# p-m-mueller/saddle_point_petsc

Measured on AMD Instinct MI355X. Metric: FGMRES iterations/sec + achieved HBM GB/s on A-block SpMV, 1/2/4/8 MI355X, higher is better.
Workload: dtype f64

## Files before the change

include/spk.h:

```cpp
#ifndef SPK_H
#define SPK_H

#include <stdint.h>

#ifdef __cplusplus
extern "C" {
#endif

#define SPK_VERSION 100

typedef struct spk_ctx spk_ctx;

enum { SPK_OK = 0, SPK_ERR_ARG = -1, SPK_ERR_HIP = -2, SPK_ERR_STATE = -3,
       SPK_ERR_COMM = -4, SPK_ERR_NOMEM = -5, SPK_ERR_UNSUPPORTED = -6 };

enum { SPK_MEM_HOST = 0, SPK_MEM_DEVICE = 1 };

enum { SPK_BLOCK_A00 = 0, SPK_BLOCK_A10 = 1 };

enum { SPK_PC_NONE = 0, SPK_PC_JACOBI = 1, SPK_PC_SCHUR = 2 };
enum { SPK_SCHUR_DIAG = 0, SPK_SCHUR_LOWER = 1, SPK_SCHUR_UPPER = 2, SPK_SCHUR_FULL = 3 };
enum { SPK_ORTHOG_CGS = 0, SPK_ORTHOG_MGS = 1 };
enum { SPK_REFINE_NEVER = 0, SPK_REFINE_IFNEEDED = 1, SPK_REFINE_ALWAYS = 2 };
enum { SPK_SPMV_CSR = 0 };
// ... 7 lines not shown
    int32_t restart;
    int32_t max_it;
    double rtol;
    double abstol;
    double dtol;
    int32_t guess_nonzero;
    int32_t orthog;
    int32_t check_every;
    int32_t fused;
    int32_t cgs_refine;
    int32_t single_reduce;
    int32_t iteration_form;
    int32_t reserved;
} spk_opts;
enum { SPK_ITER_AUTO = 0, SPK_ITER_FOUR_LAUNCH = 1, SPK_ITER_TWO_LAUNCH = 2, SPK_ITER_THREE_LAUNCH = 3, SPK_ITER_BA = 4,
       SPK_ITER_UNNORM = 5, SPK_ITER_RESIDENT = 6, SPK_ITER_LAST = 6 };

typedef struct spk_result {
    int32_t its;
    int32_t reason;
    double rnorm;
    double rnorm0;
    int32_t hist_len;
    int32_t cycles;
    double solve_seconds;
} spk_result;

int spk_create(spk_ctx **ctx, int device);
int spk_destroy(spk_ctx *ctx);
const char *spk_last_error(const spk_ctx *ctx);
int spk_version(void);
// ... 96 lines not shown
```

saddle_point_petsc_amd/csrc/spk_device.hpp:

```cpp
#pragma once
#include "spk_internal.hpp"

#include <cmath>
#include <cstdlib>

namespace spk {
namespace k {

constexpr int kThreads = 256;
constexpr int kWave = 64;
constexpr int kVT = 1024;
constexpr int kVWaves = kVT / kWave;
constexpr int kVecUnroll = 4;
constexpr int kVecMaxBlocks = 256;

__device__ __forceinline__ double wave_sum(double v)
{
#pragma unroll
    for (int off = kWave / 2; off > 0; off >>= 1) v += __shfl_down(v, off, kWave);
    return v;
}

typedef double dbl2v __attribute__((ext_vector_type(2)));
typedef int int4v __attribute__((ext_vector_type(4)));
// ... 353 lines not shown
    bool on;
};
inline WsShape ws_shape(int64_t n2)
{
    WsShape v;
    static const int knob = [] { const char *e = getenv("SPK_VEC_WS"); return e ? atoi(e) : -1; }();
    v.on = n2 < (int64_t)kVecMaxBlocks * 2048 && knob != 0;
    v.U = n2 >= (int64_t)kVecMaxBlocks * 64 * 8 ? 8 : (n2 >= (int64_t)kVecMaxBlocks * 64 * 4 ? 4 : 2);
    if (knob == 2 || knob == 4 || knob == 8) v.U = knob;
    int64_t tiles = (n2 + 64 * v.U - 1) / (64 * v.U);
    if (tiles < 1) tiles = 1;
    v.grid = (int)(tiles < kVecMaxBlocks ? tiles : kVecMaxBlocks);
    return v;
}

struct VecShape {
    int T, U, grid, G;
};
inline VecShape vec_shape(int64_t n2, bool maxpy = false)
{
    VecShape v;
    v.G = 4;
    int cap = kVecMaxBlocks;
    if (n2 >= (int64_t)kVecMaxBlocks * 2048) { v.T = 512; v.U = 4; }
    else if (n2 >= (int64_t)kVecMaxBlocks * 1024) { v.T = 256; v.U = 4; }
    else if (n2 >= (int64_t)kVecMaxBlocks * 512) { v.T = 256; v.U = 2; }
    else { v.T = 256; v.U = 1; }
    if (maxpy && n2 < (int64_t)kVecMaxBlocks * 1024) { v.T = 256; v.U = 1; v.G = 8; cap = 1024; }
    else if (maxpy && n2 < (int64_t)kVecMaxBlocks * 2048) { v.T = 256; v.U = 2; v.G = 8; cap = 1024; }
    int64_t tiles = (n2 + (int64_t)v.T * v.U - 1) / ((int64_t)v.T * v.U);
// ... 15 lines not shown
```

saddle_point_petsc_amd/csrc/spk_internal.hpp:

```cpp
#pragma once
#include <hip/hip_runtime.h>

#include <cstdint>
#include <cstdio>
#include <functional>
#include <memory>
#include <string>
#include <vector>

#include <hip/hip_ext.h>

#include "../../include/spk.h"

namespace spk {

struct Error {
    int code;
    std::string msg;
};
[[noreturn]] void fail(int code, const char *fmt, ...);

#define SPK_HIP(call)                                                                  \
    do {                                                                               \
        hipError_t e_ = (call);                                                        \
// ... 448 lines not shown
    double *c;
    const double *wl_in;
    int lam_in_dot;
    double *partials, *out;
    PeerAR ar;
    int32_t *err;
    uint32_t fin_ticks;
    SendRanges sr;
    int gmain;
    const int32_t *done;
    double *sc, *hbuf, *wl_out;
    KrylovArrays ka;
    int loc;
    int defer_fin;
};
void iter_spmv_mdot(const IterA &a, hipStream_t s, bool dots = true);
struct IterBA {
    const int32_t *browptr, *bcol;
    const double *vtop, *vbot;
    const int32_t *tile_brow;
    const int32_t *tdesc;
    int ntiles, tiles_per_xcd, slots, tb;
    int chunk;
    const int32_t *nbr, *wt;
    uint32_t *flags;
    uint32_t seq;
    const double *V;
    int64_t ldv;
    int nv;
    const double *dots;
// ... 126 lines not shown
    spk::k::Finish fin(double *out) { return spk::k::Finish{partials.p, out, spk::k::PeerAR{}, errw.p, fin_ticks}; }
    spk::k::Finish fin(double *out, const spk::k::PeerAR &ar) { return spk::k::Finish{partials.p, out, ar, errw.p, fin_ticks}; }
    void check_device_error();
    spk::DevBuf<double> y1tmp, ttmp;

    int last_form = -1, last_single = 0;

    int ws_restart = -1;
    spk::DevBuf<double> V, Z, xsol, rhs, tmp;
    spk::DevBuf<double> zun;
    spk::DevBuf<uint32_t> ba_flags;
    spk::DevBuf<double> ba_sc;
    spk::DevBuf<double> res_P;
    int num_cus = 0;
    uint32_t ba_seq = 0;
    spk::DevBuf<double> kry_d;
    spk::DevBuf<spk::KrylovState> kst;
    spk::k::KrylovArrays ka{};

    spk::DevBuf<double> stage_x, stage_y;

    void ensure_scratch();
    void ensure_vectors();
    void upload_staged(void *dst, const void *src, size_t bytes);
    void *pin_state = nullptr;
    hipEvent_t state_ev = nullptr;
    void *pin[2] = {nullptr, nullptr};
    hipEvent_t pin_ev[2] = {nullptr, nullptr};
};

// ... 12 lines not shown
```

saddle_point_petsc_amd/csrc/spk_k_iter.hip:

```cpp
#include "spk_device.hpp"

namespace spk {
namespace k {

template <int VW, int MINW>
__global__ __launch_bounds__(kThreads, MINW) void iter_spmv_mdot_kernel(IterA a)
{
    const int32_t dn = __builtin_nontemporal_load(a.done);
    __shared__ double prod[kBTile * 4];
    __shared__ double wt[kThreads], vt[kThreads];
    const double scale = a.nrm2 ? inv_norm(a.nrm2[0]) : 1.0;
    const int nmain = 8 * a.slots;
    const int nv = a.nv, m = a.m;
    const int scalar_wg = VW > 0 ? nmain : 0;
    const int bid = VW > 0 ? (int)blockIdx.x : (int)blockIdx.x - 1;
    if ((int)blockIdx.x == scalar_wg) {
        if (dn) return;
        double *lamw = wt;
        if ((int)threadIdx.x < m) {
            const int r = threadIdx.x;
            double wl;
            if (a.nrm2) {
                a.vcur[a.nl + r] *= scale;
                a.zdst[a.nl + r] = a.zsrc[a.nl + r] * scale;
// ... 195 lines not shown
    const int np = a.packed ? a.m / 2 : a.m;
    const int per = (a.nv + np + 3) / 4;
    if (a.nv + a.m > kMaxNv - 1) fail(SPK_ERR_ARG, "iter_spmv_mdot: %d values exceed one reduction", a.nv + a.m);
    static const int occ8 = [] { const char *e = getenv("SPK_ITERA_OCC"); return e ? atoi(e) : 4; }();
    const int occ = !dots ? 0 : (per <= 4 ? 4 : (per <= 8 ? (occ8 == 4 ? 4 : 3) : 2));
    a.slots = !dots ? (a.tiles_per_xcd > 0 ? a.tiles_per_xcd : 1) : iter_slots(a.tiles_per_xcd, occ);
    const dim3 grid(8 * a.slots + 1), block(kThreads);
    if (!dots) hipLaunchKernelGGL((iter_spmv_mdot_kernel<0, 4>), grid, block, 0, s, a);
    else if (per <= 4) hipLaunchKernelGGL((iter_spmv_mdot_kernel<4, 4>), grid, block, 0, s, a);
    else if (per <= 8 && occ8 == 4) hipLaunchKernelGGL((iter_spmv_mdot_kernel<8, 4>), grid, block, 0, s, a);
    else if (per <= 8) hipLaunchKernelGGL((iter_spmv_mdot_kernel<8, 3>), grid, block, 0, s, a);
    else if (per <= 12) hipLaunchKernelGGL((iter_spmv_mdot_kernel<12, 2>), grid, block, 0, s, a);
    else hipLaunchKernelGGL((iter_spmv_mdot_kernel<16, 2>), grid, block, 0, s, a);
}

template <int T, int G, int U, int MP>
__global__ __launch_bounds__(T) void iter_maxpy_uhead_kernel(IterB b)
{
    const int32_t dn = __builtin_nontemporal_load(b.done);
    __shared__ double hs[kMaxNv], lam[kMaxNv * 8], ys[8], wraws[8], tus[8];
    __shared__ double red[T];
    const int nv = b.nv, m = b.m;
    constexpr int NP = MP > 0 ? MP : 1;
    const int gmain = b.gmain;
    const int nhalo = b.sr.peer ? (2 * b.sr.nrecv + T - 1) / T : 0;
    const bool is_main = (int)blockIdx.x < gmain;
    const int64_t n2 = b.nl / 2;
    const int bid = blockIdx.x;
    const int bx = b.sr.peer ? ((bid & 1) ? gmain - 1 - (bid >> 1) : (bid >> 1)) : bid;

    constexpr bool PRE = U * (MP > 0 ? MP : 1) <= 16;
    double2 wv[U], dv[U], pe[PRE ? NP : 1][U], t0[G][U];
    int64_t idx[U];
    bool ok[U];
    int64_t tile = bx;
    auto load_planes = [&]() {
#pragma unroll
        for (int q = 0; q < NP; ++q) {
            const bool live = b.packed ? 2 * q < m : q < m;
#pragma unroll
// ... 24 lines not shown
    bool have = is_main && tile * (T * U) < n2;
    if (have) load_tile(tile);

    double lamv = 0.0;
    const bool lam_mine = (int)threadIdx.x < nv * m;
    if (lam_mine) lamv = b.V[(size_t)(threadIdx.x / m) * b.ldv + b.nl + (threadIdx.x % m)];
    double wl = 0.0, sh = 1.0;
    if ((int)threadIdx.x < m) {
        wl = b.wl_in[threadIdx.x];
        sh = b.shat[threadIdx.x];
    }
    double hi_pre = 0.0, qv_pre = 0.0, tbv_pre[8], sci = 1.0;
    const double s_w = b.sc ? b.sc[nv - 1] : 1.0;
    if (threadIdx.x < kWave) {
        const int i = threadIdx.x;
        hi_pre = i < nv ? b.dots[i] : 0.0;
        if (b.sc) sci = i < nv ? b.sc[i] : 0.0;
#pragma unroll
        for (int r = 0; r < 8; ++r) tbv_pre[r] = (r < m && i < nv) ? b.tb[i * 8 + r] : 0.0;
        qv_pre = (i < m) ? b.dots[nv + i] : 0.0;
    }
    if (dn) return;
    if (threadIdx.x < kWave) {
        const int i = threadIdx.x;
        const double hi = b.sc ? sci * s_w * hi_pre : hi_pre;
        const double ci = b.sc ? hi * sci : hi;
        double tbv[8];
#pragma unroll
        for (int r = 0; r < 8; ++r) tbv[r] = tbv_pre[r] * (b.sc ? sci : 1.0);
        const double qv = qv_pre * s_w;
        if (i < nv) hs[i] = ci;
        if (b.sc && (int)blockIdx.x == gmain + nhalo && i < nv) b.hbuf[i] = hi;
#pragma unroll
        for (int r = 0; r < 8; ++r) {
            if (r < m) {
                const double tsum = wave_sum(hi * tbv[r]);
                const double qr = __shfl(qv, r, kWave);
                if (i == 0) tus[r] = qr - tsum;
            }
        }
    }
    if (lam_mine) lam[threadIdx.x] = lamv;
    for (int t = threadIdx.x + T; t < nv * m; t += T) lam[t] = b.V[(size_t)(t / m) * b.ldv + b.nl + (t % m)];
    __syncthreads();
    if ((int)threadIdx.x < NP && MP > 0) {
        const int r = threadIdx.x;
        double y = 0.0, wraw = 0.0;
// ... 5 lines not shown
        wraws[r] = wraw;
        ys[r] = y;
    }
    __syncthreads();
    double yv[NP];
#pragma unroll
    for (int r = 0; r < NP; ++r) yv[r] = MP > 0 ? ys[r] : 0.0;
    if (b.sc && have) {
#pragma unroll
        for (int u = 0; u < U; ++u) {
            wv[u].x *= s_w;
            wv[u].y *= s_w;
        }
    }

    if ((int)blockIdx.x == gmain + nhalo) {
        if ((int)threadIdx.x < m) {
            const int r = threadIdx.x;
            double w1 = tus[r];
            if (b.fact == SPK_SCHUR_FULL)
                for (int q = 0; q < m; ++q) w1 -= b.gram[r * m + q] * ys[q];
            b.w[b.nl + r] = wraws[r];
            b.zun[b.nl + r] = ys[r];
            b.c[b.nl + r] = w1;
            b.tb[(size_t)nv * 8 + r] = tus[r];
            if (b.sc) b.wl_out[r] = w1;
        }
        __syncthreads();
        double lam2 = 0.0;
        if (threadIdx.x == 0)
            for (int r = 0; r < m; ++r) lam2 += b.lam_in_dot ? wraws[r] * wraws[r] : 0.0;
        if (b.defer_fin) {
            if (threadIdx.x == 0) publish(b.partials + (size_t)gmain * kPartialLd, lam2);
            return;
        }
        final_reduce(b.partials, gmain, kPartialLd, 1, red, FinErr{b.err, b.fin_ticks});
        if (threadIdx.x == 0) red[0] = red[0] + lam2;
        __syncthreads();
        if (b.ar.P) peer_allreduce_block(b.ar, red, 1, b.out);
        else if (threadIdx.x == 0) b.out[0] = red[0];
        return;
    }
    if (!is_main) {
        const int64_t g = (int64_t)((int)blockIdx.x - gmain) * T + threadIdx.x;
        if (g < 2 * (int64_t)b.sr.nrecv) {
            uint32_t lo;
            const unsigned long long tw0 = (b.sr.stats && threadIdx.x == 0) ? wall_clock64() : 0ull;
            const bool okw = granule_wait(b.sr.mine + g, b.sr.seq, b.sr.timeout_ms, lo, b.sr.err, b.done);
            if (b.sr.stats && threadIdx.x == 0) {
                atomicAdd(b.sr.stats + 2 * kStatHalo, wall_clock64() - tw0);
                atomicAdd(b.sr.stats + 2 * kStatHalo + 1, 1ull);
            }
            const uint32_t other = __shfl_xor(lo, 1, kWave);
            if (!(g & 1)) b.sr.xghost[g >> 1] = join_halves(lo, other);
            if (!okw) raise_comm_error(b.sr.err, 18, b.sr.seq);
        }
// ... 125 lines not shown
                    wv[u].y *= s_w;
                }
            }
        }
    }
    const int lane = threadIdx.x & 63, wave = threadIdx.x >> 6;
    const double sw = wave_sum(nrm);
    if (lane == 0) red[wave] = sw;
    __syncthreads();
    if (threadIdx.x == 0) {
        double tsum = 0.0;
#pragma unroll
        for (int j = 0; j < T / kWave; ++j) tsum += red[j];
        publish(b.partials + (size_t)bx * kPartialLd, tsum);
    }
}

int iter_maxpy_uhead(IterB b, hipStream_t s)
{
    const int64_t n2 = b.nl / 2;
    const bool thin = n2 < (int64_t)kVecMaxBlocks * 2048;
    static const int t128 = [] { const char *e = getenv("SPK_B_T128"); return e ? atoi(e) : 0; }();
    const int U = thin ? (n2 < (int64_t)kVecMaxBlocks * 1024 ? 1 : 2) : 4;
    const bool tiny = thin && U == 1 && t128 && n2 <= (int64_t)1024 * 128;
    const int T = tiny ? 128 : (thin ? 256 : 512);
    int64_t tiles = (n2 + (int64_t)T * U - 1) / ((int64_t)T * U);
    if (tiles < 1) tiles = 1;
    b.gmain = (int)std::min<int64_t>(tiles, thin ? 1024 : kVecMaxBlocks);
    int grid = b.gmain + 1;
    if (b.sr.peer) grid += (2 * b.sr.nrecv + T - 1) / T;
// ... 7 lines not shown
        if (!thin) SPK_IB(512, 4, 4, MPP);                                       \
        else if (tiny) SPK_IB(128, 8, 1, MPP);                                   \
        else if (U == 2) { if (g2 == 16) SPK_IB(256, 16, 2, MPP); else SPK_IB(256, 8, 2, MPP); } \
        else if (g1 == 32) SPK_IB(256, 32, 1, MPP);                              \
        else if (g1 == 16) SPK_IB(256, 16, 1, MPP);                              \
        else SPK_IB(256, 8, 1, MPP);                                             \
    } while (0)
    if (mp == 0) SPK_IB_MP(0);
    else if (mp == 4) SPK_IB_MP(4);
    else SPK_IB_MP(8);
#undef SPK_IB_MP
#undef SPK_IB
    return b.gmain;
}

__global__ __launch_bounds__(kWave) void tile_col_range_kernel(const int32_t *__restrict__ browptr, const int32_t *__restrict__ bcol,
                                                               const int32_t *__restrict__ tile_brow, int ntiles, int32_t *__restrict__ out)
{
    const int t = blockIdx.x;
    if (t >= ntiles) return;
    int lo = INT32_MAX, hi = -1;
    for (int q = browptr[tile_brow[t]] + (int)threadIdx.x; q < browptr[tile_brow[t + 1]]; q += kWave) {
        const int c = bcol[q];
        lo = c < lo ? c : lo;
        hi = c > hi ? c : hi;
    }
#pragma unroll
    for (int off = kWave / 2; off > 0; off >>= 1) {
        const int l2 = __shfl_down(lo, off, kWave), h2 = __shfl_down(hi, off, kWave);
        lo = l2 < lo ? l2 : lo;
// ... 339 lines not shown
```

saddle_point_petsc_amd/csrc/spk_k_vec.hip:

```cpp
#include "spk_device.hpp"

namespace spk {
namespace k {

__global__ void arm_partials_kernel(double *p, size_t n)
{
    const size_t i = (size_t)blockIdx.x * blockDim.x + threadIdx.x;
    if (i < n) p[i] = __longlong_as_double((long long)kSentinelBits);
}
void arm_partials(double *p, size_t n, hipStream_t s)
{
    hipLaunchKernelGGL(arm_partials_kernel, dim3((unsigned)((n + 255) / 256)), dim3(256), 0, s, p, n);
}

__global__ __launch_bounds__(256) void finish_probe_kernel(double *partials, double *out, FinErr fe)
{
    __shared__ double scratch[256];
    if (blockIdx.x + 1 < gridDim.x) {
        if (threadIdx.x == 0) publish(partials + (size_t)blockIdx.x * kPartialLd, 1.0);
        return;
    }
    __syncthreads();
    final_reduce(partials, gridDim.x, kPartialLd, 1, scratch, fe);
    if (threadIdx.x == 0) out[0] = scratch[0];
// ... 84 lines not shown
                       B.colidx.p, B.val.p, B.nrows, dinv, shat);
}



template <int NG, int T, int G, bool NT, int U>
__global__ __launch_bounds__(T) void mdot_kernel(const double *__restrict__ V, int64_t ldv, int nv,
                                                 const double *__restrict__ V2, int nv1,
                                                 const double *__restrict__ w, int64_t n2,
                                                 int64_t n_dot, double *__restrict__ partials,
                                                 int with_ww,
                                                 double *__restrict__ out, PeerAR ar, int split, FinErr fe,
                                                 const int32_t *__restrict__ done)
{
    if (done && *done) return;
    constexpr int NA = NG * 8 + 1, W = T / kWave, TILE2 = T * U;
    __shared__ double lds[(W * NA > T) ? W * NA : T];
    double acc[NA];
#pragma unroll
    for (int i = 0; i < NA; ++i) acc[i] = 0.0;

    for (int64_t tile = blockIdx.x; tile * TILE2 < n2; tile += gridDim.x) {
        double2 wv[U];
        int64_t idx[U];
#pragma unroll
        for (int u = 0; u < U; ++u) {
            idx[u] = tile * TILE2 + u * T + threadIdx.x;
            if (idx[u] < n2) {
                wv[u] = ld2(w, idx[u]);
                if (2 * idx[u] >= n_dot) wv[u].x = 0.0;
                if (2 * idx[u] + 1 >= n_dot) wv[u].y = 0.0;
            } else {
                wv[u].x = wv[u].y = 0.0;
                idx[u] = 0;
            }
        }
#pragma unroll
        for (int u = 0; u < U; ++u) acc[NA - 1] += wv[u].x * wv[u].x + wv[u].y * wv[u].y;
#pragma unroll
        for (int g0 = 0; g0 < NG * 8; g0 += G) {
            if (g0 < nv) {
                double2 a[G][U];
#pragma unroll
                for (int v = 0; v < G; ++v) {
                    const bool live = g0 + v < nv;
                    const int ic = live ? g0 + v : 0;
                    const int j2 = ic - nv1;
                    const double *Vi = !live ? w : (ic < nv1 ? V + (size_t)ic * ldv : V2 + (size_t)(split ? j2 >> 1 : j2) * ldv);
#pragma unroll
                    for (int u = 0; u < U; ++u) a[v][u] = ld2s<NT>(Vi, live ? idx[u] : 0);
                }
#pragma unroll
                for (int v = 0; v < G; ++v) {
                    const double mk = (g0 + v < nv) ? 1.0 : 0.0;
                    double d = 0.0;
                    if (split && g0 + v >= nv1 && g0 + v < nv) {
                        if ((g0 + v - nv1) & 1) {
#pragma unroll
                            for (int u = 0; u < U; ++u) d += a[v][u].y * wv[u].y;
                        } else {
#pragma unroll
                            for (int u = 0; u < U; ++u) d += a[v][u].x * wv[u].x;
                        }
                    } else {
#pragma unroll
                        for (int u = 0; u < U; ++u) d += a[v][u].x * wv[u].x + a[v][u].y * wv[u].y;
                    }
                    acc[g0 + v] += mk * d;
                }
            }
        }
    }
    const int lane = threadIdx.x & 63, wave = threadIdx.x >> 6;
#pragma unroll
    for (int i = 0; i < NA; ++i) {
        const double s = wave_sum(acc[i]);
        if (lane == 0) lds[wave * NA + i] = s;
    }
    __syncthreads();
    if (threadIdx.x < NA) {
        const int i = threadIdx.x;
        double s = 0.0;
#pragma unroll
        for (int j = 0; j < W; ++j) s += lds[j * NA + i];
        double *row = partials + (size_t)blockIdx.x * kPartialLd;
        if (i < nv) publish(row + i, s);
        else if (i == NA - 1 && with_ww) publish(row + nv, s);
    }
    if (!arrive_last(gridDim.x)) return;
    const int k = nv + (with_ww ? 1 : 0);
    final_reduce(partials, gridDim.x, kPartialLd, k, lds, fe);
    if (ar.P) peer_allreduce_block(ar, lds, k, out);
    else if ((int)threadIdx.x < k) out[threadIdx.x] = lds[threadIdx.x];
}

template <int VW, int U, int G, bool NT>
__global__ __launch_bounds__(256) void mdot_ws_kernel(const double *__restrict__ V, int64_t ldv, int nv,
                                                      const double *__restrict__ V2, int nv1,
                                                      const double *__restrict__ w, int64_t n2, int64_t n_dot,
                                                      double *__restrict__ partials, int with_ww, double *__restrict__ out,
                                                      PeerAR ar, int split, FinErr fe, const int32_t *__restrict__ done)
{
    if (done && *done) return;
// ... 800 lines not shown
```

saddle_point_petsc_amd/csrc/spk_ksp.cpp:

```cpp
#include <cstdio>
#include <cstdlib>
#include <cstring>
#include <string>
#include <vector>

#include "../../include/spk_ksp.h"

struct SpkKSP_s {
    spk_ctx *ctx = nullptr;
    int device = 0;
    spk_opts opts;
    int32_t pc_type = SPK_PC_NONE, schur_fact = SPK_SCHUR_FULL;
    int32_t inner_sweeps = 0;
    double inner_omega = 1.0;
    bool inner_richardson = false;
    bool have_ops = false, is_setup = false, has_B = false;
    bool ksp_type_given = false, pc_type_given = false;
    bool monitor = false, print_reason = false, view = false;
    spk_result result;
    std::vector<double> history;
    std::string err;
};

namespace {
// ... 192 lines not shown
        } else if (key == "-fieldsplit_0_ksp_max_it" || key == "-spk_inner_sweeps") {
            if (!val || !parse_int(val, &k->inner_sweeps)) return need("an integer");
            if (key == "-spk_inner_sweeps") k->inner_richardson = k->inner_sweeps > 0;
        } else if (key == "-fieldsplit_0_ksp_richardson_scale" || key == "-spk_inner_omega") {
            if (!val || !parse_double(val, &k->inner_omega)) return need("a real");
        } else if (key == "-fieldsplit_1_ksp_type") {
            if (!val) return need("a type");
            if (std::string(val) != "preonly") return bad();
        } else if (key == "-fieldsplit_0_pc_type" || key == "-fieldsplit_1_pc_type") {
            if (!val) return need("a type");
            if (std::string(val) != "jacobi") return bad();
        } else if (key == "-spk_single_reduce") {
            if (!val || !parse_int(val, &k->opts.single_reduce)) return need("an integer (0 off, 1 on)");
        } else if (key == "-spk_iteration_form") {
            if (!val || !parse_int(val, &k->opts.iteration_form) || k->opts.iteration_form < 0 || k->opts.iteration_form > SPK_ITER_LAST)
                return need("an integer 0..5 (0 automatic, 1 four / 2 two / 3 three launches per iteration, 4 BA, 5 three launches on an un-normalised basis)");
        } else if (key == "-spk_check_every") {
            if (!val || !parse_int(val, &k->opts.check_every)) return need("an integer");
        } else if (key.rfind("-ksp_", 0) == 0 || key.rfind("-pc_", 0) == 0 || key.rfind("-fieldsplit_", 0) == 0) {
            return set_err(k, SPK_ERR_UNSUPPORTED, "unknown solver option " + key);
        }
    }
    k->is_setup = false;
    return SPK_OK;
}

int SpkKSPSetUp(SpkKSP k)
{
    if (!k) return SPK_ERR_ARG;
    if (!k->ksp_type_given)
        return set_err(k, SPK_ERR_UNSUPPORTED, "KSPSetUp: no -ksp_type given; PETSc's default (gmres, left preconditioning) is "
// ... 63 lines not shown
```

saddle_point_petsc_amd/csrc/spk_solver.cpp:

```cpp
#include <algorithm>
#include <chrono>
#include <cstddef>
#include <cstdlib>
#include <cstring>
#include <numeric>

#include "spk_internal.hpp"

using namespace spk;

void spk_ctx::ensure_scratch()
{
    if (!partials.p) {
        partials.alloc((size_t)k::kMaxBlocks * k::kPartialLd);
        k::arm_partials(partials.p, partials.n, stream);
        SPK_HIP(hipStreamSynchronize(stream));
    }
    if (!errw.p) errw.alloc(4);
    if (!small.p) small.alloc(512);
    if (!y1tmp.p) y1tmp.alloc(64);
    if (!ttmp.p) ttmp.alloc(64);
}

void spk_ctx::check_device_error()
{
    if (!errw.p) return;
    int32_t e = 0;
    SPK_HIP(hipMemcpy(&e, errw.p, sizeof e, hipMemcpyDeviceToHost));
    if (!e) return;
    SPK_HIP(hipStreamSynchronize(stream));
    SPK_HIP(hipMemset(errw.p, 0, sizeof(int32_t)));
    k::arm_partials(partials.p, partials.n, stream);
    SPK_HIP(hipStreamSynchronize(stream));
    fail(SPK_ERR_HIP, "a cross-workgroup reduction timed out on the device (a workgroup never published its partial "
                      "sums within %.1f s): execution failure, the result of this call is not valid", fin_ticks / 1e8);
}

void spk_ctx::ensure_vectors()
{
    const int64_t want = ((int64_t)n_local + m + 255) / 256 * 256;
    if (want != ld) {
        ld = want;
        ws_restart = -1;
        tmp.release();
        zun.release();
        tmpb.release();
        bt_cached = nullptr;
        stage_x.release();
        stage_y.release();
        xsol.release();
// ... 1184 lines not shown
    const int bpk = fused && c->bd_packed ? 1 : 0;
    const double *bdp = fused ? (bpk ? c->bdpk.p : c->bd.p) : nullptr;
    const bool single = head && o.orthog == SPK_ORTHOG_CGS && o.cgs_refine == SPK_REFINE_NEVER &&
                        o.single_reduce == 1 && mk + c->m <= k::kMaxNv - 1;

    int form = o.iteration_form;
    if (const char *e = getenv("SPK_ITER_FORM")) {
        char *end = nullptr;
        const long f = strtol(e, &end, 10);
        if (end == e || *end || f < SPK_ITER_AUTO || f > SPK_ITER_LAST)
            fail(SPK_ERR_ARG, "SPK_ITER_FORM=%s: not an iteration form (%d..%d)", e, (int)SPK_ITER_AUTO, (int)SPK_ITER_LAST);
        form = (int)f;
    }
    if (form < SPK_ITER_AUTO || form > SPK_ITER_LAST) fail(SPK_ERR_ARG, "fgmres: unknown iteration_form %d", form);
    const bool un3 = head && !single && o.orthog == SPK_ORTHOG_CGS && o.cgs_refine == SPK_REFINE_NEVER &&
                     mk + c->m <= k::kMaxNv - 2 && (form == SPK_ITER_UNNORM || form == SPK_ITER_AUTO || form == SPK_ITER_RESIDENT);
    static const bool res_env_off = [] { const char *e = getenv("SPK_RESIDENT"); return e && !strcmp(e, "0"); }();
    const int res_planes = !fused ? 0 : (bpk ? m / 2 : m);
    const bool res_multi = c->comm->size() > 1;
    const bool res_rank_ok = !res_multi ? (c->peers.empty() && c->n_ghost == 0)
                                        : (c->res_fit_all && c->comm->fuses() && (c->peers.empty() || c->send_ranges.n > 0));
    const bool resident = un3 && (form == SPK_ITER_RESIDENT || (form == SPK_ITER_AUTO && !res_env_off)) && res_rank_ok &&
                          c->spmv_format == 1 && c->Adict.ok && c->Adict.bs == 2 && nl % 2 == 0 && mk >= (res_multi ? 3 : 2) &&
                          k::resident_fits(c->Adict, c->num_cus, mk, res_planes);
    if (resident) {
        const size_t need = (size_t)k::resident_scratch_doubles(c->num_cus, mk);
        if (c->res_P.n < need) c->res_P.alloc(need);
    }
    const bool two_ok = head && !single && o.orthog == SPK_ORTHOG_CGS && o.cgs_refine == SPK_REFINE_NEVER &&
                        c->spmv_format == 1 && c->Ab.ok && !c->Ab.long_rows && mk + c->m <= k::kMaxNv - 2;
    const bool two = two_ok && !un3 && (form == SPK_ITER_TWO_LAUNCH || form == SPK_ITER_THREE_LAUNCH);
    const bool three = two && form != SPK_ITER_TWO_LAUNCH;
    const bool ba = two_ok && form == SPK_ITER_BA && c->Ab.ba_ok && c->peers.empty() && c->comm->size() == 1 &&
                    (c->m <= 4 || 8 * c->Ab.ba_slots + 1 <= 512);
    if (ba) {
        const size_t nfl = (size_t)(8 * c->Ab.ba_slots + 1) * 32;
        if (c->ba_flags.n < nfl) {
            c->ba_flags.alloc(nfl);
            c->ba_seq = 0;
        }
    }
    if (ba || un3) {
        if (c->ba_sc.n < (size_t)mk + 2) c->ba_sc.alloc((size_t)mk + 2);
    }
    if (two && c->zun.n < (size_t)ld) c->zun.alloc((size_t)ld);
    const int lam_in_dot = c->comm->rank() == 0 ? 1 : 0;
    c->last_form = resident ? SPK_ITER_RESIDENT : ba ? SPK_ITER_BA : un3 ? SPK_ITER_UNNORM : two ? (three ? SPK_ITER_THREE_LAUNCH : SPK_ITER_TWO_LAUNCH)
                   : head ? SPK_ITER_FOUR_LAUNCH : -1;
    c->last_single = single ? 1 : 0;

    c->ka.tentative = single ? 1 : 0;
    KrylovState st{};
    int32_t errword = 0;
    int cycles = 0;
    if (!c->pin_state) SPK_HIP(hipHostMalloc(&c->pin_state, 512, hipHostMallocDefault));
    if (!c->state_ev) SPK_HIP(hipEventCreateWithFlags(&c->state_ev, hipEventDisableTiming));
    KrylovState *ps = (KrylovState *)c->pin_state;
    int32_t *pe = (int32_t *)((char *)c->pin_state + 384);
    pe[0] = pe[1] = 0;
    bool pend_check = false;
    bool finished = false;
    const int kAhead = 2;
// ... 70 lines not shown
                    r.shat = c->shat.p; r.gram = c->gram.p; r.P = c->res_P.p; r.ka = c->ka; r.sc_out = c->ba_sc.p;
                    r.err = c->errw.p; r.ticks = c->fin_ticks;
                    r.sr0 = k::SendRanges{};
                    r.sr1 = k::SendRanges{};
                    if (res_multi) {
                        r.sr0 = c->send_ranges;
                        r.sr1 = c->send_ranges;
                        if (!c->comm->resident_plan(mk + 1, c->peers.empty() ? 0 : mk - 1, r.ar, r.sr0, r.sr1, c->xghost.p))
                            fail(SPK_ERR_COMM, "fgmres: the communicator cannot carry a resident cycle (agreed at set-up, refused now)");
                        if (c->peers.empty()) r.sr0.n = r.sr1.n = 0;
                        if (c->n_ghost > 0) r.od = c->offdiag();
                    }
                    if (!k::cycle_resident(c->Adict, c->num_cus, r, done, s)) fail(SPK_ERR_STATE, "fgmres: resident cycle kernel refused its shape");
                    break;
                }
                {
                    const bool one = loc + 1 + m <= 40;
                    const bool spl = bpk && one;
                    const k::PeerAR ar = one ? c->comm->fused_allreduce(loc + 2 + (fused ? m : 0), k::kStatArDots) : k::PeerAR{};
                    k::mdot(V, ld, loc + 1, w, N, n_dot, c->fin(db, ar), done, s, fused ? (spl ? c->bdpk.p : c->bd.p) : nullptr,
                            fused ? m : 0, spl ? 1 : 0);
                    if (!ar.P) c->comm->allreduce_sum(db, loc + 2 + (fused ? m : 0), s);
                }
                if (un3) {
                    const k::PeerAR ar2 = c->comm->fused_allreduce(1, k::kStatArNorm);
                    k::IterB b{};
                    b.V = V; b.ldv = ld; b.nv = loc + 1; b.dots = db; b.tb = c->ka.tb;
                    b.w = w; b.dinv = c->dinv.p; b.bd = bdp; b.ldb = ld; b.shat = c->shat.p; b.gram = c->gram.p;
                    b.fact = fused ? c->schur_fact : SPK_SCHUR_LOWER;
                    b.nl = nl; b.m = m; b.packed = bpk;
                    b.zun = Zj(loc + 1); b.c = fused ? Vj(loc + 2) : nullptr; b.wl_in = wl(loc); b.wl_out = wl(loc + 1);
                    b.lam_in_dot = lam_in_dot;
                    b.partials = c->partials.p; b.out = nb; b.ar = ar2; b.err = c->errw.p; b.fin_ticks = c->fin_ticks;
                    b.sc = c->ba_sc.p; b.hbuf = sm2; b.ka = c->ka; b.loc = loc;
                    const bool defer = loc + 1 < mk && (c->comm->size() == 1 || ar2.P);
                    b.defer_fin = defer ? 1 : 0;
                    k::SendRanges sr = c->send_ranges;
                    const bool inb = sr.n > 0 && c->comm->fused_halo(sr, c->xghost.p);
                    if (sr.n > 0) b.sr = sr;
                    b.done = done;
                    const int fin_n = k::iter_maxpy_uhead(b, s);
                    if (!ar2.P && !defer) c->comm->allreduce_sum(nb, 1, s);
                    k::GivensRider gr{c->ka, loc, sm2, nb, c->ba_sc.p, defer ? c->partials.p : nullptr, defer ? fin_n : 0,
                                      k::FinErr{c->errw.p, c->fin_ticks}, defer ? ar2 : k::PeerAR{}};
                    if (loc + 1 < mk) product(Zj(loc + 1), Vj(loc + 2), inb, &gr);
                    else pend_h = sm2, pend_n = nb, pend_loc = loc;
                    last = -1;
                }
                if (ba) {
                k::IterBA p{};
                p.browptr = c->Ab.browptr.p; p.bcol = c->Ab.bcol.p; p.vtop = c->Ab.vtop.p; p.vbot = c->Ab.vbot.p;
                p.tile_brow = c->Ab.tile_brow.p; p.ntiles = c->Ab.ntiles; p.tiles_per_xcd = (c->Ab.ntiles + 7) / 8;
                p.slots = c->Ab.ba_slots; p.tb = c->Ab.ba_tb; p.chunk = c->Ab.ba_chunk; p.nbr = nullptr; p.wt = c->Ab.ba_wt.p;
                p.tdesc = c->Ab.tile_desc.p;
                p.flags = c->ba_flags.p; p.seq = ++c->ba_seq;
                p.V = V; p.ldv = ld; p.nv = loc + 1; p.dots = db; p.sc = c->ba_sc.p; p.tb_ = c->ka.tb;
// ... 238 lines not shown
```

Baseline: 6204.

## Fuse Gram-Schmidt MDot and MAXPY into one launch on single rank

Adds a new iteration form in which the multi-dot product and the MAXPY/norm update of each unnormalised-basis FGMRES step run in a single kernel. The last-arriving workgroup reduces the dot partials and publishes the totals to a double-buffered sentinel array, and the other workgroups spin-wait on it before doing the MAXPY part. This removes one launch and a kernel boundary per Arnoldi step. It is only used on one rank without ghosts, and only when occupancy guarantees that all workgroups are co-resident. It risks busy-wait stalls and a larger register footprint in the fused kernel.

```diff
diff --git a/include/spk.h b/include/spk.h
--- a/include/spk.h
+++ b/include/spk.h
@@ -45,7 +45,8 @@
     int32_t reserved;
 } spk_opts;
 enum { SPK_ITER_AUTO = 0, SPK_ITER_FOUR_LAUNCH = 1, SPK_ITER_TWO_LAUNCH = 2, SPK_ITER_THREE_LAUNCH = 3, SPK_ITER_BA = 4,
-       SPK_ITER_UNNORM = 5, SPK_ITER_RESIDENT = 6, SPK_ITER_LAST = 6 };
+       SPK_ITER_UNNORM = 5, SPK_ITER_RESIDENT = 6, SPK_ITER_GS_FUSED = 7,
+       SPK_ITER_LAST = 7 };
 
 typedef struct spk_result {
     int32_t its;
diff --git a/saddle_point_petsc_amd/csrc/spk_device.hpp b/saddle_point_petsc_amd/csrc/spk_device.hpp
--- a/saddle_point_petsc_amd/csrc/spk_device.hpp
+++ b/saddle_point_petsc_amd/csrc/spk_device.hpp
@@ -391,6 +391,87 @@
     return v;
 }
 
+template <int NG, int T, int G, bool NT, int U>
+__device__ __forceinline__ void mdot_tiles(const double *__restrict__ V, int64_t ldv, int nv,
+                                           const double *__restrict__ V2, int nv1,
+                                           const double *__restrict__ w, int64_t n2,
+                                           int64_t n_dot, double *__restrict__ partials,
+                                           int with_ww, int split, double *lds)
+{
+    constexpr int NA = NG * 8 + 1, W = T / kWave, TILE2 = T * U;
+    double acc[NA];
+#pragma unroll
+    for (int i = 0; i < NA; ++i) acc[i] = 0.0;
+
+    for (int64_t tile = blockIdx.x; tile * TILE2 < n2; tile += gridDim.x) {
+        double2 wv[U];
+        int64_t idx[U];
+#pragma unroll
+        for (int u = 0; u < U; ++u) {
+            idx[u] = tile * TILE2 + u * T + threadIdx.x;
+            if (idx[u] < n2) {
+                wv[u] = ld2(w, idx[u]);
+                if (2 * idx[u] >= n_dot) wv[u].x = 0.0;
+                if (2 * idx[u] + 1 >= n_dot) wv[u].y = 0.0;
+            } else {
+                wv[u].x = wv[u].y = 0.0;
+                idx[u] = 0;
+            }
+        }
+#pragma unroll
+        for (int u = 0; u < U; ++u) acc[NA - 1] += wv[u].x * wv[u].x + wv[u].y * wv[u].y;
+#pragma unroll
+        for (int g0 = 0; g0 < NG * 8; g0 += G) {
+            if (g0 < nv) {
+                double2 a[G][U];
+#pragma unroll
+                for (int v = 0; v < G; ++v) {
+                    const bool live = g0 + v < nv;
+                    const int ic = live ? g0 + v : 0;
+                    const int j2 = ic - nv1;
+                    const double *Vi = !live ? w : (ic < nv1 ? V + (size_t)ic * ldv : V2 + (size_t)(split ? j2 >> 1 : j2) * ldv);
+#pragma unroll
+                    for (int u = 0; u < U; ++u) a[v][u] = ld2s<NT>(Vi, live ? idx[u] : 0);
+                }
+#pragma unroll
+                for (int v = 0; v < G; ++v) {
+                    const double mk = (g0 + v < nv) ? 1.0 : 0.0;
+                    double d = 0.0;
+                    if (split && g0 + v >= nv1 && g0 + v < nv) {
+                        if ((g0 + v - nv1) & 1) {
+#pragma unroll
+                            for (int u = 0; u < U; ++u) d += a[v][u].y * wv[u].y;
+                        } else {
+#pragma unroll
+                            for (int u = 0; u < U; ++u) d += a[v][u].x * wv[u].x;
+                        }
+                    } else {
+#pragma unroll
+                        for (int u = 0; u < U; ++u) d += a[v][u].x * wv[u].x + a[v][u].y * wv[u].y;
+                    }
+                    acc[g0 + v] += mk * d;
+                }
+            }
+        }
+    }
+    const int lane = threadIdx.x & 63, wave = threadIdx.x >> 6;
+#pragma unroll
+    for (int i = 0; i < NA; ++i) {
+        const double s = wave_sum(acc[i]);
+        if (lane == 0) lds[wave * NA + i] = s;
+    }
+    __syncthreads();
+    if (threadIdx.x < NA) {
+        const int i = threadIdx.x;
+        double s = 0.0;
+#pragma unroll
+        for (int j = 0; j < W; ++j) s += lds[j * NA + i];
+        double *row = partials + (size_t)blockIdx.x * kPartialLd;
+        if (i < nv) publish(row + i, s);
+        else if (i == NA - 1 && with_ww) publish(row + nv, s);
+    }
+}
+
 struct VecShape {
     int T, U, grid, G;
 };
diff --git a/saddle_point_petsc_amd/csrc/spk_internal.hpp b/saddle_point_petsc_amd/csrc/spk_internal.hpp
--- a/saddle_point_petsc_amd/csrc/spk_internal.hpp
+++ b/saddle_point_petsc_amd/csrc/spk_internal.hpp
@@ -486,6 +486,18 @@
     int loc;
     int defer_fin;
 };
+struct GsArgs {
+    const double *V2;
+    int cnt, split;
+    int64_t n2, n_dot;
+    double *partials;
+    double *out;
+    double *tot, *tot_next;
+    FinErr fe;
+};
+int gs_fused(IterB b, GsArgs g, hipStream_t s);
+int gs_fused_occupancy(int ng, int m);
+int64_t gs_fused_grid(int64_t nl);
 void iter_spmv_mdot(const IterA &a, hipStream_t s, bool dots = true);
 struct IterBA {
     const int32_t *browptr, *bcol;
@@ -642,6 +654,10 @@
     spk::DevBuf<double> res_P;
     int num_cus = 0;
     uint32_t ba_seq = 0;
+    spk::DevBuf<double> gs_tot;
+    uint32_t gs_seq = 0;
+    int gs_occ[3] = {-1, -1, -1};
+    bool gs_fused_fits(int64_t nl, int m);
     spk::DevBuf<double> kry_d;
     spk::DevBuf<spk::KrylovState> kst;
     spk::k::KrylovArrays ka{};
diff --git a/saddle_point_petsc_amd/csrc/spk_k_iter.hip b/saddle_point_petsc_amd/csrc/spk_k_iter.hip
--- a/saddle_point_petsc_amd/csrc/spk_k_iter.hip
+++ b/saddle_point_petsc_amd/csrc/spk_k_iter.hip
@@ -233,8 +233,8 @@
     else hipLaunchKernelGGL((iter_spmv_mdot_kernel<16, 2>), grid, block, 0, s, a);
 }
 
-template <int T, int G, int U, int MP>
-__global__ __launch_bounds__(T) void iter_maxpy_uhead_kernel(IterB b)
+template <int T, int G, int U, int MP, class Dots>
+__device__ __forceinline__ void maxpy_uhead_tiles(const IterB &b, int scalar_wg, Dots dots)
 {
     const int32_t dn = __builtin_nontemporal_load(b.done);
     __shared__ double hs[kMaxNv], lam[kMaxNv * 8], ys[8], wraws[8], tus[8];
@@ -242,7 +242,6 @@
     const int nv = b.nv, m = b.m;
     constexpr int NP = MP > 0 ? MP : 1;
     const int gmain = b.gmain;
-    const int nhalo = b.sr.peer ? (2 * b.sr.nrecv + T - 1) / T : 0;
     const bool is_main = (int)blockIdx.x < gmain;
     const int64_t n2 = b.nl / 2;
     const int bid = blockIdx.x;
@@ -297,11 +296,11 @@
     const double s_w = b.sc ? b.sc[nv - 1] : 1.0;
     if (threadIdx.x < kWave) {
         const int i = threadIdx.x;
-        hi_pre = i < nv ? b.dots[i] : 0.0;
+        hi_pre = i < nv ? dots(i) : 0.0;
         if (b.sc) sci = i < nv ? b.sc[i] : 0.0;
 #pragma unroll
         for (int r = 0; r < 8; ++r) tbv_pre[r] = (r < m && i < nv) ? b.tb[i * 8 + r] : 0.0;
-        qv_pre = (i < m) ? b.dots[nv + i] : 0.0;
+        qv_pre = (i < m) ? dots(nv + i) : 0.0;
     }
     if (dn) return;
     if (threadIdx.x < kWave) {
@@ -313,7 +312,7 @@
         for (int r = 0; r < 8; ++r) tbv[r] = tbv_pre[r] * (b.sc ? sci : 1.0);
         const double qv = qv_pre * s_w;
         if (i < nv) hs[i] = ci;
-        if (b.sc && (int)blockIdx.x == gmain + nhalo && i < nv) b.hbuf[i] = hi;
+        if (b.sc && (int)blockIdx.x == scalar_wg && i < nv) b.hbuf[i] = hi;
 #pragma unroll
         for (int r = 0; r < 8; ++r) {
             if (r < m) {
@@ -349,7 +348,7 @@
         }
     }
 
-    if ((int)blockIdx.x == gmain + nhalo) {
+    if ((int)blockIdx.x == scalar_wg) {
         if ((int)threadIdx.x < m) {
             const int r = threadIdx.x;
             double w1 = tus[r];
@@ -367,14 +366,15 @@
             for (int r = 0; r < m; ++r) lam2 += b.lam_in_dot ? wraws[r] * wraws[r] : 0.0;
         if (b.defer_fin) {
             if (threadIdx.x == 0) publish(b.partials + (size_t)gmain * kPartialLd, lam2);
+            if (!is_main) return;
+        } else {
+            final_reduce(b.partials, gmain, kPartialLd, 1, red, FinErr{b.err, b.fin_ticks});
+            if (threadIdx.x == 0) red[0] = red[0] + lam2;
+            __syncthreads();
+            if (b.ar.P) peer_allreduce_block(b.ar, red, 1, b.out);
+            else if (threadIdx.x == 0) b.out[0] = red[0];
             return;
         }
-        final_reduce(b.partials, gmain, kPartialLd, 1, red, FinErr{b.err, b.fin_ticks});
-        if (threadIdx.x == 0) red[0] = red[0] + lam2;
-        __syncthreads();
-        if (b.ar.P) peer_allreduce_block(b.ar, red, 1, b.out);
-        else if (threadIdx.x == 0) b.out[0] = red[0];
-        return;
     }
     if (!is_main) {
         const int64_t g = (int64_t)((int)blockIdx.x - gmain) * T + threadIdx.x;
@@ -530,6 +530,12 @@
         for (int j = 0; j < T / kWave; ++j) tsum += red[j];
         publish(b.partials + (size_t)bx * kPartialLd, tsum);
     }
+}
+template <int T, int G, int U, int MP>
+__global__ __launch_bounds__(T) void iter_maxpy_uhead_kernel(IterB b)
+{
+    const int nhalo = b.sr.peer ? (2 * b.sr.nrecv + T - 1) / T : 0;
+    maxpy_uhead_tiles<T, G, U, MP>(b, b.gmain + nhalo, [&](int i) { return b.dots[i]; });
 }
 
 int iter_maxpy_uhead(IterB b, hipStream_t s)
@@ -567,6 +573,87 @@
     return b.gmain;
 }
 
+struct TotalsWait {
+    const double *tot;
+    FinErr fe;
+    __device__ double operator()(int i) const
+    {
+        double v = peek(tot + i);
+        if (is_sentinel(v)) {
+            const unsigned long long t0 = wall_clock64();
+            do {
+                __builtin_amdgcn_s_sleep(1);
+                v = peek(tot + i);
+            } while (is_sentinel(v) && wall_clock64() - t0 < (unsigned long long)fe.ticks &&
+                     !(fe.err && __hip_atomic_load(fe.err, __ATOMIC_RELAXED, __HIP_MEMORY_SCOPE_AGENT)));
+            if (is_sentinel(v) && fe.err) __hip_atomic_store(fe.err, 1, __ATOMIC_RELAXED, __HIP_MEMORY_SCOPE_AGENT);
+        }
+        return v;
+    }
+};
+
+constexpr int kGsT = 512, kGsU = 4, kGsG = 4;
+
+template <int NG, int MP>
+__global__ __launch_bounds__(kGsT) void gs_fused_kernel(IterB b, GsArgs g)
+{
+    constexpr int NA = NG * 8 + 1, W = kGsT / kWave;
+    __shared__ double lds[(W * NA > kGsT) ? W * NA : kGsT];
+    if (blockIdx.x == 0 && threadIdx.x < kWave) publish(g.tot_next + threadIdx.x, __longlong_as_double((long long)kSentinelBits));
+    if (*b.done) return;
+    mdot_tiles<NG, kGsT, kGsG, true, kGsU>(b.V, b.ldv, g.cnt, g.V2, b.nv, b.w, g.n2, g.n_dot, g.partials, 1, g.split, lds);
+    if (arrive_last(gridDim.x)) {
+        const int k = g.cnt + 1;
+        final_reduce(g.partials, gridDim.x, kPartialLd, k, lds, g.fe);
+        if ((int)threadIdx.x < k) {
+            g.out[threadIdx.x] = lds[threadIdx.x];
+            publish(g.tot + threadIdx.x, lds[threadIdx.x]);
+        }
+    }
+    maxpy_uhead_tiles<kGsT, kGsG, kGsU, MP>(b, (int)gridDim.x - 2, TotalsWait{g.tot, g.fe});
+}
+
+#define SPK_GS_SWITCH(NGV, MPV, CASE)                                                        \
+    switch ((NGV) * 10 + (MPV)) {                                                           \
+    case 10: CASE(1, 0); case 20: CASE(2, 0); case 30: CASE(3, 0); case 40: CASE(4, 0); case 50: CASE(5, 0); \
+    case 14: CASE(1, 4); case 24: CASE(2, 4); case 34: CASE(3, 4); case 44: CASE(4, 4); case 54: CASE(5, 4); \
+    case 18: CASE(1, 8); case 28: CASE(2, 8); case 38: CASE(3, 8); case 48: CASE(4, 8); default: CASE(5, 8); \
+    }
+
+int gs_fused_occupancy(int ng, int m)
+{
+    const int mp = m == 0 ? 0 : (m <= 4 ? 4 : 8);
+    int nb = 0;
+#define SPK_GS_OCC(NG, MP) SPK_HIP(hipOccupancyMaxActiveBlocksPerMultiprocessor(&nb, gs_fused_kernel<NG, MP>, kGsT, 0)); break
+    SPK_GS_SWITCH(ng, mp, SPK_GS_OCC)
+#undef SPK_GS_OCC
+    return nb;
+}
+
+int64_t gs_fused_grid(int64_t nl)
+{
+    const int64_t n2 = nl / 2;
+    if (n2 < (int64_t)kVecMaxBlocks * 2048) return 0;
+    return kVecMaxBlocks;
+}
+
+int gs_fused(IterB b, GsArgs g, hipStream_t s)
+{
+    const int64_t grid = gs_fused_grid(b.nl);
+    const VecShape vs = vec_shape(g.n2);
+    if (!grid || vs.T != kGsT || vs.U != kGsU || vs.grid != grid) fail(SPK_ERR_STATE, "gs_fused: not the fat vector shape");
+    if (!b.defer_fin || b.ar.P || b.sr.n || b.sr.peer) fail(SPK_ERR_STATE, "gs_fused: one rank, norm reduced by the rider only");
+    if (g.cnt > 40 || b.nv + b.m > kMaxNv - 1) fail(SPK_ERR_ARG, "gs_fused: %d values exceed one reduction", g.cnt);
+    b.gmain = (int)grid;
+    const int ng = (g.cnt + 7) / 8 > 0 ? (g.cnt + 7) / 8 : 1;
+    const int mp = b.m == 0 ? 0 : (b.m <= 4 ? 4 : 8);
+#define SPK_GS_LAUNCH(NG, MP) hipLaunchKernelGGL((gs_fused_kernel<NG, MP>), dim3((unsigned)grid), dim3(kGsT), 0, s, b, g); break
+    SPK_GS_SWITCH(ng, mp, SPK_GS_LAUNCH)
+#undef SPK_GS_LAUNCH
+    return b.gmain;
+}
+#undef SPK_GS_SWITCH
+
 __global__ __launch_bounds__(kWave) void tile_col_range_kernel(const int32_t *__restrict__ browptr, const int32_t *__restrict__ bcol,
                                                                const int32_t *__restrict__ tile_brow, int ntiles, int32_t *__restrict__ out)
 {
diff --git a/saddle_point_petsc_amd/csrc/spk_k_vec.hip b/saddle_point_petsc_amd/csrc/spk_k_vec.hip
--- a/saddle_point_petsc_amd/csrc/spk_k_vec.hip
+++ b/saddle_point_petsc_amd/csrc/spk_k_vec.hip
@@ -122,79 +122,9 @@
                                                  const int32_t *__restrict__ done)
 {
     if (done && *done) return;
-    constexpr int NA = NG * 8 + 1, W = T / kWave, TILE2 = T * U;
+    constexpr int NA = NG * 8 + 1, W = T / kWave;
     __shared__ double lds[(W * NA > T) ? W * NA : T];
-    double acc[NA];
-#pragma unroll
-    for (int i = 0; i < NA; ++i) acc[i] = 0.0;
-
-    for (int64_t tile = blockIdx.x; tile * TILE2 < n2; tile += gridDim.x) {
-        double2 wv[U];
-        int64_t idx[U];
-#pragma unroll
-        for (int u = 0; u < U; ++u) {
-            idx[u] = tile * TILE2 + u * T + threadIdx.x;
-            if (idx[u] < n2) {
-                wv[u] = ld2(w, idx[u]);
-                if (2 * idx[u] >= n_dot) wv[u].x = 0.0;
-                if (2 * idx[u] + 1 >= n_dot) wv[u].y = 0.0;
-            } else {
-                wv[u].x = wv[u].y = 0.0;
-                idx[u] = 0;
-            }
-        }
-#pragma unroll
-        for (int u = 0; u < U; ++u) acc[NA - 1] += wv[u].x * wv[u].x + wv[u].y * wv[u].y;
-#pragma unroll
-        for (int g0 = 0; g0 < NG * 8; g0 += G) {
-            if (g0 < nv) {
-                double2 a[G][U];
-#pragma unroll
-                for (int v = 0; v < G; ++v) {
-                    const bool live = g0 + v < nv;
-                    const int ic = live ? g0 + v : 0;
-                    const int j2 = ic - nv1;
-                    const double *Vi = !live ? w : (ic < nv1 ? V + (size_t)ic * ldv : V2 + (size_t)(split ? j2 >> 1 : j2) * ldv);
-#pragma unroll
-                    for (int u = 0; u < U; ++u) a[v][u] = ld2s<NT>(Vi, live ? idx[u] : 0);
-                }
-#pragma unroll
-                for (int v = 0; v < G; ++v) {
-                    const double mk = (g0 + v < nv) ? 1.0 : 0.0;
-                    double d = 0.0;
-                    if (split && g0 + v >= nv1 && g0 + v < nv) {
-                        if ((g0 + v - nv1) & 1) {
-#pragma unroll
-                            for (int u = 0; u < U; ++u) d += a[v][u].y * wv[u].y;
-                        } else {
-#pragma unroll
-                            for (int u = 0; u < U; ++u) d += a[v][u].x * wv[u].x;
-                        }
-                    } else {
-#pragma unroll
-                        for (int u = 0; u < U; ++u) d += a[v][u].x * wv[u].x + a[v][u].y * wv[u].y;
-                    }
-                    acc[g0 + v] += mk * d;
-                }
-            }
-        }
-    }
-    const int lane = threadIdx.x & 63, wave = threadIdx.x >> 6;
-#pragma unroll
-    for (int i = 0; i < NA; ++i) {
-        const double s = wave_sum(acc[i]);
-        if (lane == 0) lds[wave * NA + i] = s;
-    }
-    __syncthreads();
-    if (threadIdx.x < NA) {
-        const int i = threadIdx.x;
-        double s = 0.0;
-#pragma unroll
-        for (int j = 0; j < W; ++j) s += lds[j * NA + i];
-        double *row = partials + (size_t)blockIdx.x * kPartialLd;
-        if (i < nv) publish(row + i, s);
-        else if (i == NA - 1 && with_ww) publish(row + nv, s);
-    }
+    mdot_tiles<NG, T, G, NT, U>(V, ldv, nv, V2, nv1, w, n2, n_dot, partials, with_ww, split, lds);
     if (!arrive_last(gridDim.x)) return;
     const int k = nv + (with_ww ? 1 : 0);
     final_reduce(partials, gridDim.x, kPartialLd, k, lds, fe);
diff --git a/saddle_point_petsc_amd/csrc/spk_ksp.cpp b/saddle_point_petsc_amd/csrc/spk_ksp.cpp
--- a/saddle_point_petsc_amd/csrc/spk_ksp.cpp
+++ b/saddle_point_petsc_amd/csrc/spk_ksp.cpp
@@ -230,7 +230,8 @@
             if (!val || !parse_int(val, &k->opts.single_reduce)) return need("an integer (0 off, 1 on)");
         } else if (key == "-spk_iteration_form") {
             if (!val || !parse_int(val, &k->opts.iteration_form) || k->opts.iteration_form < 0 || k->opts.iteration_form > SPK_ITER_LAST)
-                return need("an integer 0..5 (0 automatic, 1 four / 2 two / 3 three launches per iteration, 4 BA, 5 three launches on an un-normalised basis)");
+                return need("an integer 0..7 (0 automatic, 1 four / 2 two / 3 three launches per iteration, 4 BA, 5 three launches on an "
+                            "un-normalised basis, 6 one launch per restart cycle, 7 as 5 with MDot and MAXPY in one launch)");
         } else if (key == "-spk_check_every") {
             if (!val || !parse_int(val, &k->opts.check_every)) return need("an integer");
         } else if (key.rfind("-ksp_", 0) == 0 || key.rfind("-pc_", 0) == 0 || key.rfind("-fieldsplit_", 0) == 0) {
diff --git a/saddle_point_petsc_amd/csrc/spk_solver.cpp b/saddle_point_petsc_amd/csrc/spk_solver.cpp
--- a/saddle_point_petsc_amd/csrc/spk_solver.cpp
+++ b/saddle_point_petsc_amd/csrc/spk_solver.cpp
@@ -31,9 +31,23 @@
     SPK_HIP(hipStreamSynchronize(stream));
     SPK_HIP(hipMemset(errw.p, 0, sizeof(int32_t)));
     k::arm_partials(partials.p, partials.n, stream);
+    if (gs_tot.p) k::arm_partials(gs_tot.p, gs_tot.n, stream);
     SPK_HIP(hipStreamSynchronize(stream));
     fail(SPK_ERR_HIP, "a cross-workgroup reduction timed out on the device (a workgroup never published its partial "
                       "sums within %.1f s): execution failure, the result of this call is not valid", fin_ticks / 1e8);
+}
+
+bool spk_ctx::gs_fused_fits(int64_t nl, int m)
+{
+    const int64_t grid = k::gs_fused_grid(nl);
+    if (!grid) return false;
+    const int mi = m == 0 ? 0 : (m <= 4 ? 1 : 2);
+    if (gs_occ[mi] < 0) {
+        int occ = 1 << 30;
+        for (int ng = 1; ng <= 5; ++ng) occ = std::min(occ, k::gs_fused_occupancy(ng, m));
+        gs_occ[mi] = occ;
+    }
+    return (int64_t)gs_occ[mi] * num_cus >= grid;
 }
 
 void spk_ctx::ensure_vectors()
@@ -1248,7 +1262,8 @@
     }
     if (form < SPK_ITER_AUTO || form > SPK_ITER_LAST) fail(SPK_ERR_ARG, "fgmres: unknown iteration_form %d", form);
     const bool un3 = head && !single && o.orthog == SPK_ORTHOG_CGS && o.cgs_refine == SPK_REFINE_NEVER &&
-                     mk + c->m <= k::kMaxNv - 2 && (form == SPK_ITER_UNNORM || form == SPK_ITER_AUTO || form == SPK_ITER_RESIDENT);
+                     mk + c->m <= k::kMaxNv - 2 &&
+                     (form == SPK_ITER_UNNORM || form == SPK_ITER_AUTO || form == SPK_ITER_RESIDENT || form == SPK_ITER_GS_FUSED);
     static const bool res_env_off = [] { const char *e = getenv("SPK_RESIDENT"); return e && !strcmp(e, "0"); }();
     const int res_planes = !fused ? 0 : (bpk ? m / 2 : m);
     const bool res_multi = c->comm->size() > 1;
@@ -1261,6 +1276,12 @@
         const size_t need = (size_t)k::resident_scratch_doubles(c->num_cus, mk);
         if (c->res_P.n < need) c->res_P.alloc(need);
     }
+    const bool gsf = un3 && !resident && (form == SPK_ITER_GS_FUSED || form == SPK_ITER_AUTO) && c->comm->size() == 1 &&
+                     c->peers.empty() && c->n_ghost == 0 && mk + m <= 41 && c->gs_fused_fits(nl, m);
+    if (gsf && !c->gs_tot.p) {
+        c->gs_tot.alloc(2 * k::kPartialLd);
+        k::arm_partials(c->gs_tot.p, c->gs_tot.n, s);
+    }
     const bool two_ok = head && !single && o.orthog == SPK_ORTHOG_CGS && o.cgs_refine == SPK_REFINE_NEVER &&
                         c->spmv_format == 1 && c->Ab.ok && !c->Ab.long_rows && mk + c->m <= k::kMaxNv - 2;
     const bool two = two_ok && !un3 && (form == SPK_ITER_TWO_LAUNCH || form == SPK_ITER_THREE_LAUNCH);
@@ -1279,7 +1300,7 @@
     }
     if (two && c->zun.n < (size_t)ld) c->zun.alloc((size_t)ld);
     const int lam_in_dot = c->comm->rank() == 0 ? 1 : 0;
-    c->last_form = resident ? SPK_ITER_RESIDENT : ba ? SPK_ITER_BA : un3 ? SPK_ITER_UNNORM : two ? (three ? SPK_ITER_THREE_LAUNCH : SPK_ITER_TWO_LAUNCH)
+    c->last_form = resident ? SPK_ITER_RESIDENT : gsf ? SPK_ITER_GS_FUSED : ba ? SPK_ITER_BA : un3 ? SPK_ITER_UNNORM : two ? (three ? SPK_ITER_THREE_LAUNCH : SPK_ITER_TWO_LAUNCH)
                    : head ? SPK_ITER_FOUR_LAUNCH : -1;
     c->last_single = single ? 1 : 0;
 
@@ -1380,7 +1401,8 @@
                     if (!k::cycle_resident(c->Adict, c->num_cus, r, done, s)) fail(SPK_ERR_STATE, "fgmres: resident cycle kernel refused its shape");
                     break;
                 }
-                {
+                const bool gs = gsf && loc + 1 < mk;
+                if (!gs) {
                     const bool one = loc + 1 + m <= 40;
                     const bool spl = bpk && one;
                     const k::PeerAR ar = one ? c->comm->fused_allreduce(loc + 2 + (fused ? m : 0), k::kStatArDots) : k::PeerAR{};
@@ -1405,7 +1427,23 @@
                     const bool inb = sr.n > 0 && c->comm->fused_halo(sr, c->xghost.p);
                     if (sr.n > 0) b.sr = sr;
                     b.done = done;
-                    const int fin_n = k::iter_maxpy_uhead(b, s);
+                    int fin_n;
+                    if (gs) {
+                        k::GsArgs g{};
+                        g.V2 = fused ? (bpk ? c->bdpk.p : c->bd.p) : nullptr;
+                        g.cnt = loc + 1 + (fused ? m : 0);
+                        g.split = bpk;
+                        g.n2 = (N + 1) / 2; g.n_dot = n_dot;
+                        g.partials = c->partials.p + 1;
+                        g.out = db;
+                        g.tot = c->gs_tot.p + (c->gs_seq & 1) * k::kPartialLd;
+                        g.tot_next = c->gs_tot.p + ((c->gs_seq + 1) & 1) * k::kPartialLd;
+                        g.fe = k::FinErr{c->errw.p, c->fin_ticks};
+                        fin_n = k::gs_fused(b, g, s);
+                        ++c->gs_seq;
+                    } else {
+                        fin_n = k::iter_maxpy_uhead(b, s);
+                    }
                     if (!ar2.P && !defer) c->comm->allreduce_sum(nb, 1, s);
                     k::GivensRider gr{c->ka, loc, sm2, nb, c->ba_sc.p, defer ? c->partials.p : nullptr, defer ? fin_n : 0,
                                       k::FinErr{c->errw.p, c->fin_ticks}, defer ? ar2 : k::PeerAR{}};
```

After: 6450 (median of 6 runs). +4.0%, better.
